# rneddojr/Adapting-Pretrained-Vision-Transformers-with-LoRA-against-Attack-Vectors

Hardware: AMD Instinct MI355X
Metric: adversarial images/sec (PGD-20, ViT-B/16+LoRA r=8, bs256) (higher is better)
Workload: dtype f16; 1 GPU; PGD-20 eps=8/255 alpha=2/255 random_start, ViT-B/16 (21 classes) + LoRA r=8 on q,k,v,attn-out,fc2 (fused), batch 256/GPU of synthetic 224x224x3 in HBM, seeded random-init weights; global_batch=256, per_gpu_batch=256, scaling=weak, pgd_steps=20, lora_rank=8, parallelism=dp1 (batch shards, no data-path collective), ranks_seen_by_collective=1

## Files before the change

adapting-pretrained-vision-transformers-with-lora-against-attack-vectors_amd/csrc/cls_path.hip:

```cpp
#include "kernels.h"
#include "prof.h"

namespace VLNS {

namespace {

constexpr int HD = 64;

__device__ __forceinline__ float row8_sum(float v) {
    v += __shfl_xor(v, 1, 64); v += __shfl_xor(v, 2, 64); return v + __shfl_xor(v, 4, 64);
}
__device__ __forceinline__ float slot8_sum(float v) {
    v += __shfl_xor(v, 8, 64); v += __shfl_xor(v, 16, 64); return v + __shfl_xor(v, 32, 64);
}
__device__ __forceinline__ float slot8_max(float v) {
    v = fmaxf(v, __shfl_xor(v, 8, 64)); v = fmaxf(v, __shfl_xor(v, 16, 64)); return fmaxf(v, __shfl_xor(v, 32, 64));
}
__device__ __forceinline__ void cvt8(const h16x8& t, float (&v)[8]) {
#pragma unroll
    for (int k = 0; k < 8; ++k) v[k] = h2f(t[k]);
}

__global__ __launch_bounds__(256) void attn_cls_fwd_kernel(const h16* __restrict__ qkv, h16* __restrict__ ctx_c,
                                                           float* __restrict__ lse_c, int B, int T, int H, int D,
// ... 120 lines not shown
    if (i >= (int64_t)B * n4) return;
    const int b = (int)(i / n4), c = (int)(i - (int64_t)b * n4);
    const h16x4 v = *(const h16x4*)(src + b * stride + 4 * c);
    *(f32x4*)(dst + (int64_t)b * D + 4 * c) = f32x4{h2f(v[0]), h2f(v[1]), h2f(v[2]), h2f(v[3])};
}
__global__ __launch_bounds__(256) void scatter_rows_kernel(const float* __restrict__ src, h16* __restrict__ dst, int B, int D,
                                                           int64_t stride) {
    const int n4 = D / 4;
    const int64_t i = blockIdx.x * (int64_t)blockDim.x + threadIdx.x;
    if (i >= (int64_t)B * n4) return;
    const int b = (int)(i / n4), c = (int)(i - (int64_t)b * n4);
    const f32x4 v = *(const f32x4*)(src + (int64_t)b * D + 4 * c);
    *(h16x4*)(dst + b * stride + 4 * c) = h16x4{f2h_sat(v[0]), f2h_sat(v[1]), f2h_sat(v[2]), f2h_sat(v[3])};
}

}

int k_attn_cls_fwd(const h16* qkv, h16* ctx_c, float* lse_c, int B, int T, int H, int D, hipStream_t s) {
    if (T > 256 || D != H * HD) return -1;
    ProfScope prof_("attn_cls_fwd_kernel", 4.0 * B * H * (double)T * HD, (double)B * T * D * 4.0, s);
    hipLaunchKernelGGL(attn_cls_fwd_kernel, dim3((B * H + 3) / 4), dim3(256), 0, s, qkv, ctx_c, lse_c, B, T, H, D,
                       0.125f * 1.4426950408889634f);
    return 0;
}
int k_attn_cls_bwd(const h16* qkv, const h16* ctx_c, const h16* dctx_c, const float* lse_c, h16* dqkv, int B, int T, int H, int D,
                   hipStream_t s) {
    if (T > 256 || D != H * HD) return -1;
    ProfScope prof_("attn_cls_bwd_kernel", 10.0 * B * H * (double)T * HD, (double)B * T * D * 10.0, s);
    hipLaunchKernelGGL(attn_cls_bwd_kernel, dim3((B * H + 3) / 4), dim3(256), 0, s, qkv, ctx_c, dctx_c, lse_c, dqkv, B, T, H, D,
                       0.125f, 0.125f * 1.4426950408889634f);
    return 0;
}
void k_gather_rows(const h16* src, float* dst, int B, int D, int64_t stride, hipStream_t s) {
    const int64_t n = (int64_t)B * (D / 4);
    hipLaunchKernelGGL(gather_rows_kernel, dim3((unsigned)((n + 255) / 256)), dim3(256), 0, s, src, dst, B, D, stride);
}
void k_scatter_rows(const float* src, h16* dst, int B, int D, int64_t stride, hipStream_t s) {
    const int64_t n = (int64_t)B * (D / 4);
    hipLaunchKernelGGL(scatter_rows_kernel, dim3((unsigned)((n + 255) / 256)), dim3(256), 0, s, src, dst, B, D, stride);
}

}
```

adapting-pretrained-vision-transformers-with-lora-against-attack-vectors_amd/csrc/kernels.h:

```cpp
#pragma once
#include "common.h"
#include "gemm.h"

namespace VLNS {

void k_patch_gather(const float* x, h16* out, int B, int S, int P, int normalise, const float* mean,
                    const float* std, hipStream_t s);
void k_cls_rows(float* x, const float* cls, const float* pos, int B, int T, int D, hipStream_t s);
void k_layernorm_fwd(const float* x, h16* h, float* mean, float* rstd, const float* g, const float* b, int M, int D,
                     float eps, const h16* delta, float* xout, const h16* P, int ng, h16* t, hipStream_t s,
                     int ldh = 0);
void k_layernorm_bwd(const h16* dh, const float* x, const float* mean, const float* rstd, const float* g,
                     const float* dres, float* dx, h16* dx_h, int M, int D, const h16* P, int ng, h16* u, hipStream_t s,
                     int* err = nullptr, int ldh = 0);
void k_head_fwd(const float* x, int B, int T, int D, int C, float eps, const float* g, const float* b, const float* Wc,
                const float* bc, float* xhat, float* xf, float* rstd, float* logits, hipStream_t s);
void k_cls_rows16(h16* x, const float* cls, const float* pos, int B, int T, int D, hipStream_t s);
void k_layernorm_fwd16(const h16* x, h16* h, float* mean, float* rstd, const float* g, const float* b, int M, int D,
                       float eps, const h16* delta, h16* xout, const h16* P, int ng, h16* t, hipStream_t s, int* err = nullptr);
void k_layernorm_bwd16(const h16* dh, const h16* x, const float* mean, const float* rstd, const float* g, h16* dres, int M, int D,
                       const h16* P, int ng, h16* u, hipStream_t s, int* err = nullptr);
void k_head_fwd16(const h16* x, int B, int T, int D, int C, float eps, const float* g, const float* b, const float* Wc,
                  const float* bc, float* xhat, float* xf, float* rstd, float* logits, hipStream_t s);
void k_ce_loss(const float* logits, const int64_t* labels, int B, int C, float* dlogits, float* loss_img, float* loss,
// ... 79 lines not shown

void attention32_set_ring(int on);
int attention32_init(int device);
int k_attention32_fwd(const h16* qkv, h16* ctx, float* lse2, int B, int T, int H, int D, hipStream_t s);
int k_attention32_bwd(const h16* qkv, const h16* ctx, const h16* dctx, const float* lse2, h16* dqkv, int B, int T,
                      int H, int D, hipStream_t s);

int k_attention_img_fwd(const h16* qkv, h16* ctx, float* lse2, int B, int T, int H, int D, const h16* Ad, h16* t, int r,
                        hipStream_t s);
int k_attention_img_bwd(const h16* qkv, const h16* ctx, const h16* dctx, const float* lse2, h16* dqkv, int B, int T, int H,
                        int D, const h16* Bd, h16* u, int r, unsigned mods, hipStream_t s, int force_ring = -1);

int k_attn_cls_fwd(const h16* qkv, h16* ctx_c, float* lse_c, int B, int T, int H, int D, hipStream_t s);
int k_attn_cls_bwd(const h16* qkv, const h16* ctx_c, const h16* dctx_c, const float* lse_c, h16* dqkv, int B, int T, int H, int D,
                   hipStream_t s);
void k_gather_rows(const h16* src, float* dst, int B, int D, int64_t stride, hipStream_t s);
void k_scatter_rows(const float* src, h16* dst, int B, int D, int64_t stride, hipStream_t s);

void k_patch_overlay(const float* img, const float* patch, const float* mats, const float* persp, float* out, int B, int S,
                     int ps, int circle, hipStream_t s);
void k_patch_overlay_bwd(const float* g, const float* mats, const float* persp, float* dpatch, int B, int S, int ps, int circle,
                         hipStream_t s);
void k_clamp(float* x, float lo, float hi, int64_t n, hipStream_t s);

int lora_wgrad_chunk(int M);
int lora_wgrad_chunks(int M);
void k_lora_wgrad(const h16* L, int ldl, int ncols_l, const h16* Rm, int ldr, int ncols_r, int M, float scale,
                  float* out, int ldo, int transpose_out, const float* inv_gscale, int64_t chunk_stride, hipStream_t s);
void k_reduce_chunks(const float* slab, float* out, int64_t n, int chunks, int64_t stride, hipStream_t s);

// ... 2 lines not shown
```

adapting-pretrained-vision-transformers-with-lora-against-attack-vectors_amd/csrc/model.h:

```cpp
#pragma once
#include <cstddef>
#include <string>
#include <vector>

#include "common.h"
#define vl_model VL_API(vl_model)
#include "../../include/vitlora.h"
#include "kernels.h"

enum { LQKV = 0, LO = 1, LFC1 = 2, LFC2 = 3 };
static const uint32_t kTargetBits[6] = {VL_T_Q, VL_T_K, VL_T_V, VL_T_O, VL_T_FC1, VL_T_FC2};

namespace VLNS {

struct Slot {
    int target_idx;
    int row_off;
    int out, in;
    int ext_off;
    int64_t a_off, b_off;
};

struct Linear {
    int out = 0, in = 0;
// ... 30 lines not shown
    std::vector<h16*> t[4];
    float *xhat, *xf, *rstd_f, *logits, *dlogits, *loss, *loss_img;
    float *gscale, *inv_gscale;
    float* dres[2];
    h16 *dres_h;
    h16 *dh, *dctx, *dqkv, *dz, *u;
    h16* xd;
    float* wg_slab;
    float* grad_img;
    struct Cls {
        int64_t Bc = 0;
        float *x0, *x1, *x2, *mean, *rstd, *lse;
        h16 *ctx, *delta, *h2, *a, *z, *t;
        float* dres[2];
        h16 *dres_h, *dh, *dctx, *dz, *u;
    } c;
    float *stage_x0, *stage_adv;
    int64_t* stage_labels;
    float* f_patches;
    std::vector<float*> f_h1, f_h2, f_a, f_qkv, f_ctx, f_z;
    std::vector<float*> f_t[4];
    float *f_dh, *f_dctx, *f_dqkv, *f_dz, *f_u, *f_xd, *f_tmp;
};

struct Pass {
    Workspace ws;
    int B = 0, rows = 0;
    int norm = 0, train = 0, cls_only = 0, have_loss = 0;
};

// ... 43 lines not shown
    hipStream_t cap_stream = nullptr;
    static constexpr int CHAIN_MAX_BATCH = 191;
    VLNS::Pass half[2];
    int chain_batch = 0;
    int pgd_chains = 0;
    hipStream_t side_stream = nullptr;
    hipEvent_t ev_fork = nullptr, ev_join = nullptr;
    int api_chains = 0;
    int fwd_chains = 0;
    int64_t n_captures = 0, n_commits = 0;
    int use_graph = 1;
    int resid_epi = 2;
    int plan_batch = 0, plan_train = 0;
    int attn_img_mode = -1;
    int num_cus = 256;
    int dead_rows = 1;
    int fuse_down_min_k = 2048;
    int small_m_rows = 16384;
    int fuse_pgd = 1;
    int square_bare = 0;
    int* err_flag = nullptr;
    float mean[3] = {0.485f, 0.456f, 0.406f};
    float stdv[3] = {0.229f, 0.224f, 0.225f};
};

static_assert(offsetof(vl_model, cfg) == 0, "api_dispatch.cpp reads the precision through the vl_config the handle starts with");

int vl_fail(int code, const char* fmt, ...);
#define HIPCHK(expr)                                                                            \
    do {                                                                                        \
// ... 40 lines not shown
```

adapting-pretrained-vision-transformers-with-lora-against-attack-vectors_amd/csrc/vitlora.hip:

```cpp
#include <algorithm>
#include <cstdarg>
#include <cstdio>
#include <cstdlib>
#include <cstring>
#include <string>
#include <vector>

#include "common.h"
#include "env.h"
#include "api_rename.h"
#include "model.h"
#include "prof.h"

extern std::vector<VlFlatRecord> g_vl_models;
extern long long g_poison_count;
#ifndef VL_BF16
Profiler* g_prof = nullptr;
int g_poison_lds = 0;
long long g_poison_count = 0;
namespace {
__global__ __launch_bounds__(256) void poison_lds_kernel(unsigned pattern, unsigned* sink) {
    extern __shared__ unsigned lds_all[];
    constexpr int N = 160 * 1024 / 4;
    for (int i = threadIdx.x; i < N; i += 256) lds_all[i] = pattern;
// ... 139 lines not shown
            launch_gemm(main, EPI_STORE_H16, 128, s);
            GemmArgs lo = gemm_args(u, ln.kext, ln.Au, ln.kext, ln.kext, Mpad, ln.in);
            lo.Mvalid = Mvalid; lo.k2_algo = 0;
            lo.C = g.C; lo.ldc = g.ldc; lo.R = p.ws.xd; lo.ldr = ln.in;
            if (epi == EPI_GELU_BWD) { lo.G = (const h16*)g.R; lo.ldg = g.ldr; }
            lo.drop_seed = m->drop_seed; lo.drop_stream = stream_id; lo.drop_p = m->cfg.lora_dropout;
            lo.drop_inv_keep = 1.f / (1.f - m->cfg.lora_dropout);
            launch_gemm(lo, EPI_DROP_ACC, 128, s);
            return;
        }
        g.k2_algo = m->r * (int)ln.slots.size();
        g.k2_used = ext_cols(m, ln);
        add_ext(g, u, ln.kext, ln.Au, ln.kext, ln.kext);
    }
    launch_gemm(g, epi, 128, s);
}

int parse_layer(const char* name, const char** rest) {
    const char* pfx = "vit.encoder.layer.";
    const size_t n = strlen(pfx);
    if (strncmp(name, pfx, n) != 0) return -1;
    char* end = nullptr;
    long i = strtol(name + n, &end, 10);
    if (end == name + n || *end != '.') return -1;
    *rest = end + 1;
    return (int)i;
}

bool capturing(hipStream_t s) {
    hipStreamCaptureStatus st = hipStreamCaptureStatusNone;
// ... 75 lines not shown
    if (int e = gemm_init(dev)) return fail(VL_ERR_HIP, "gemm_init: hipFuncSetAttribute failed (%d) on device %d", e, dev);
    if (int e = attention32_init(dev)) return fail(VL_ERR_HIP, "attention32_init: hipFuncSetAttribute failed (%d) on device %d", e, dev);
    if (int e = f32_init(dev)) return fail(VL_ERR_HIP, "f32_init: hipFuncSetAttribute failed (%d) on device %d", e, dev);
    vl_model* m = new vl_model();
    m->cfg = *cfg;
    m->device = dev;
    m->f32 = cfg->precision == VL_PREC_F32;
    m->D = cfg->hidden; m->L = cfg->layers; m->H = cfg->heads; m->MLP = cfg->mlp;
    m->S = cfg->image_size; m->P = cfg->patch_size; m->G = G; m->NP = G * G; m->T = G * G + 1;
    m->C = cfg->num_labels; m->PK = 3 * cfg->patch_size * cfg->patch_size;
    m->r = cfg->lora_targets ? cfg->lora_r : 0;
    m->scaling = m->r ? cfg->lora_alpha / (float)m->r : 0.f;
    m->use_graph = !env_flag("VITLORA_NO_GRAPH", false);
    m->resid_epi = env_resid();
    m->dead_rows = env_flag("VITLORA_DEAD_ROWS", true);
    m->fuse_pgd = env_flag("VITLORA_FUSE_PGD", true);
    m->pgd_chains = std::min(std::max(env_int("VITLORA_PGD_CHAINS", m->pgd_chains), 0), 2);
    m->fuse_down_min_k = env_int("VITLORA_FUSE_DOWN_MIN_K", m->fuse_down_min_k);
    m->small_m_rows = env_int("VITLORA_SMALL_M_ROWS", m->small_m_rows);
    m->attn_img_mode = env_attn_img();
    { hipDeviceProp_t prop; m->num_cus = hipGetDeviceProperties(&prop, dev) == hipSuccess ? prop.multiProcessorCount : 256; }
    const int D = m->D, MLP = m->MLP, r = m->r;
    int rc;
#define A_(p, n) if ((rc = dev_alloc(m, &(p), (size_t)(n))) != VL_OK) { vl_destroy(m); return rc; }
    const bool f32 = m->f32;
    if (f32) { A_(m->Wpe_f32, (size_t)D * m->PK); } else { A_(m->Wpe, (size_t)D * m->PK); A_(m->WpeT, (size_t)m->PK * D); }
    A_(m->bpe, D); A_(m->cls, D);
    A_(m->pos, (size_t)m->T * D); A_(m->lnf_g, D); A_(m->lnf_b, D);
    int64_t off = 0;
    m->layers.resize(m->L);
// ... 199 lines not shown
    m->dirty = 1;
    return VL_OK;
}

int vl_merge_weight(vl_model* m, int layer, uint32_t target, const float* W_in, float* W_out, void* stream) {
    if (!m || !W_in || !W_out) return fail(VL_ERR_ARG, "null argument");
    if (layer < 0 || layer >= m->L) return fail(VL_ERR_ARG, "layer out of range");
    for (int k = 0; k < 4; ++k)
        for (const Slot& sl : m->layers[layer].lin[k].slots)
            if (kTargetBits[sl.target_idx] == target) {
                k_merge_f32(W_in, m->flat + sl.a_off, m->flat + sl.b_off, sl.out, sl.in, m->r, m->scaling, W_out,
                            (hipStream_t)stream);
                return VL_OK;
            }
    return fail(VL_ERR_ARG, "target 0x%x has no adapter in layer %d", target, layer);
}

static size_t carve(const vl_model* m, Workspace& w, int B, int train, char* base) {
    const int D = m->D, L = m->L, MLP = m->MLP;
    const int64_t Mpad = pad_rows(m, B), Mppad = pad_patch_rows(m, B);
    Carver cv{base, 0};
    w.base = base; w.max_batch = base ? B : 0; w.train = train;
    w.Mpad = Mpad; w.Mppad = Mppad;
    w.xs.assign(2 * L + 1, nullptr); w.xs16.assign(2 * L + 1, nullptr);
    if (m->f32) for (auto& p : w.xs) p = cv.take<float>((size_t)Mpad * D * 4);
    else for (auto& p : w.xs16) p = cv.take<h16>((size_t)Mpad * D * 2);
    w.mean.resize(2 * L); w.rstd.resize(2 * L);
    for (int i = 0; i < 2 * L; ++i) { w.mean[i] = cv.take<float>(Mpad * 4); w.rstd[i] = cv.take<float>(Mpad * 4); }
    w.lse.resize(L);
    for (int l = 0; l < L; ++l) w.lse[l] = cv.take<float>((size_t)B * m->H * m->T * 4);
// ... 36 lines not shown
        c.lse = cv.take<float>((size_t)B * m->H * 4);
        c.ctx = cv.take<h16>((size_t)Bc * D * 2); c.delta = cv.take<h16>((size_t)Bc * D * 2); c.h2 = cv.take<h16>((size_t)Bc * D * 2);
        c.a = cv.take<h16>((size_t)Bc * MLP * 2); c.z = cv.take<h16>((size_t)Bc * MLP * 2);
        c.t = cv.take<h16>((size_t)Bc * kext_max * 2);
        c.dres[0] = cv.take<float>((size_t)Bc * D * 4); c.dres[1] = cv.take<float>((size_t)Bc * D * 4);
        c.dres_h = cv.take<h16>((size_t)Bc * D * 2); c.dh = cv.take<h16>((size_t)Bc * D * 2); c.dctx = cv.take<h16>((size_t)Bc * D * 2);
        c.dz = cv.take<h16>((size_t)Bc * MLP * 2); c.u = cv.take<h16>((size_t)Bc * kext_max * 2);
    }
    w.dres_h = cv.take<h16>((size_t)Mpad * D * 2);
    w.dh = cv.take<h16>((size_t)Mpad * D * 2);
    w.dctx = cv.take<h16>((size_t)Mpad * D * 2);
    w.dqkv = cv.take<h16>((size_t)Mpad * 3 * D * 2);
    w.dz = cv.take<h16>((size_t)Mpad * MLP * 2);
    w.u = cv.take<h16>((size_t)Mpad * kext_max * 2);
    w.xd = train ? cv.take<h16>((size_t)Mpad * MLP * 2) : nullptr;
    w.wg_slab = train && m->cls_w_off > 0 ? cv.take<float>((size_t)lora_wgrad_chunks((int)((int64_t)B * m->T)) * (size_t)m->cls_w_off * 4) : nullptr;
    return w.bytes = cv.off;
}
static size_t carve_bytes(const vl_model* m, int B, int train) {
    Workspace scratch;
    return carve(m, scratch, B, train, nullptr);
}

static int chain_images(const vl_model* m, int max_batch) {
    if (m->f32 || m->pgd_chains == 1 || max_batch < 2) return 0;
    const int top = max_batch < vl_model::CHAIN_MAX_BATCH ? max_batch : vl_model::CHAIN_MAX_BATCH;
    return (top + 1) / 2;
}

int vl_plan(vl_model* m, int max_batch, int train, size_t* bytes) {
// ... 49 lines not shown
        p.B = B; p.norm = normalise; p.have_loss = 0;
        return VL_OK;
    }
    k_patch_gather(x, w.patches, B, m->S, m->P, normalise, m->mean, m->stdv, s);
    {
        GemmArgs g = gemm_args(w.patches, m->PK, m->Wpe, m->PK, m->PK, Mppad, D);
        g.Mvalid = B * m->NP; g.bias = m->bpe; g.C = w.xs16[0]; g.ldc = D;
        g.pos = m->pos; g.tokens = T; g.patches = m->NP;
        launch_gemm(g, EPI_PATCH_FWD, 128, s);
    }
    k_cls_rows16(w.xs16[0], m->cls, m->pos, B, T, D, s);
    h16* delta = w.dres_h;
    int* const ef = m->err_flag;
    const bool re = m->resid_epi >= 1, re2 = m->resid_epi >= 2;
    const bool cls_only = m->dead_rows && !train;
    for (int l = 0; l < L; ++l) {
        Layer& ly = m->layers[l];
        GemmArgs g;
        const int n1 = fused_down_fwd(m, p, ly.lin[LQKV]);
        const h16* P1 = n1 ? ly.lin[LQKV].Ad : nullptr;
        if (l == 0 || re2) k_layernorm_fwd16(w.xs16[2 * l], w.h1[l], w.mean[2 * l], w.rstd[2 * l], ly.ln1_g, ly.ln1_b, M, D, m->cfg.ln_eps, nullptr, nullptr, P1, n1, w.t[LQKV][l], s, ef);
        else k_layernorm_fwd16(w.xs16[2 * l - 1], w.h1[l], w.mean[2 * l], w.rstd[2 * l], ly.ln1_g, ly.ln1_b, M, D, m->cfg.ln_eps, delta, w.xs16[2 * l], P1, n1, w.t[LQKV][l], s, ef);
        memset(&g, 0, sizeof g); g.C = w.qkv[l]; g.ldc = 3 * D;
        linear_fwd(m, p, ly.lin[LQKV], w.h1[l], w.t[LQKV][l], Mpad, M, g, EPI_STORE_H16, s, l * 4 + LQKV, n1 > 0);
        if (cls_only && l == L - 1) {
            Workspace::Cls& c = w.c;
            const int Bc = (int)c.Bc;
            if (k_attn_cls_fwd(w.qkv[l], c.ctx, c.lse, B, T, m->H, D, s)) return fail(VL_ERR_UNSUPPORTED, "attention: T > 256");
            memset(&g, 0, sizeof g); g.C = c.delta; g.ldc = D;
            linear_fwd(m, p, ly.lin[LO], c.ctx, c.t, Bc, B, g, EPI_STORE_H16, s, l * 4 + LO);
            k_gather_rows(w.xs16[2 * l], c.x0, B, D, (int64_t)T * D, s);
            const int n2c = fused_down_fwd(m, p, ly.lin[LFC1]);
            k_layernorm_fwd(c.x0, c.h2, c.mean, c.rstd, ly.ln2_g, ly.ln2_b, B, D, m->cfg.ln_eps, c.delta, c.x1,
                            n2c ? ly.lin[LFC1].Ad : nullptr, n2c, c.t, s);
            memset(&g, 0, sizeof g); g.C = c.a; g.ldc = m->MLP; g.C2 = c.z; g.ldc2 = m->MLP;
            linear_fwd(m, p, ly.lin[LFC1], c.h2, c.t, Bc, B, g, EPI_GELU, s, l * 4 + LFC1, n2c > 0);
            memset(&g, 0, sizeof g); g.C = c.delta; g.ldc = D;
            linear_fwd(m, p, ly.lin[LFC2], c.a, c.t, Bc, B, g, EPI_STORE_H16, s, l * 4 + LFC2);
            k_layernorm_fwd(c.x1, nullptr, nullptr, nullptr, nullptr, nullptr, B, D, m->cfg.ln_eps, c.delta, c.x2, nullptr, 0, nullptr, s);
            k_head_fwd(c.x2, B, 1, D, m->C, m->cfg.ln_eps, m->lnf_g, m->lnf_b, m->flat + m->cls_w_off,
                       m->flat + m->cls_b_off, w.xhat, w.xf, w.rstd_f, w.logits, s);
            p.B = B; p.norm = normalise; p.have_loss = 0; p.cls_only = 1;
            return VL_OK;
        }
        const bool img = attn_img(m, B);
        const bool t_o = img && down_fusable(m, ly.lin[LO]) && !vl_drop_on(m, p);
        if (img) {
            if (k_attention_img_fwd(w.qkv[l], w.ctx[l], w.lse[l], B, T, m->H, D, t_o ? ly.lin[LO].Ad : nullptr, w.t[LO][l], m->r, s))
                return fail(VL_ERR_UNSUPPORTED, "attention: T > 224");
        } else if (k_attention32_fwd(w.qkv[l], w.ctx[l], w.lse[l], B, T, m->H, D, s)) return fail(VL_ERR_UNSUPPORTED, "attention: T > 224");
        memset(&g, 0, sizeof g); g.C = delta; g.ldc = D;
        if (re) { g.C = w.xs16[2 * l + 1]; g.R = w.xs16[2 * l]; g.ldr = D; }
        linear_fwd(m, p, ly.lin[LO], w.ctx[l], w.t[LO][l], Mpad, M, g, re ? EPI_RESID_H16 : EPI_STORE_H16, s, l * 4 + LO, t_o);
        const int n2 = fused_down_fwd(m, p, ly.lin[LFC1]);
        const h16* P2 = n2 ? ly.lin[LFC1].Ad : nullptr;
        if (re) k_layernorm_fwd16(w.xs16[2 * l + 1], w.h2[l], w.mean[2 * l + 1], w.rstd[2 * l + 1], ly.ln2_g, ly.ln2_b, M, D, m->cfg.ln_eps, nullptr, nullptr, P2, n2, w.t[LFC1][l], s, ef);
        else k_layernorm_fwd16(w.xs16[2 * l], w.h2[l], w.mean[2 * l + 1], w.rstd[2 * l + 1], ly.ln2_g, ly.ln2_b, M, D, m->cfg.ln_eps, delta, w.xs16[2 * l + 1], P2, n2, w.t[LFC1][l], s, ef);
// ... 94 lines not shown
    for (int l = L - 1; l >= 0; --l) {
        Layer& ly = m->layers[l];
        GemmArgs g;
        if (cls_only && l == L - 1) {
            Workspace::Cls& c = w.c;
            const int Bc = (int)c.Bc;
            k_head_bwd(w.dlogits, w.gscale, m->flat + m->cls_w_off, m->lnf_g, w.xhat, w.rstd_f, B, 1, D, m->C, c.dres[0], c.dres_h, s);
            memset(&g, 0, sizeof g); g.C = c.dz; g.ldc = MLP; g.R = c.z; g.ldr = MLP;
            linear_dgrad(m, p, ly.lin[LFC2], c.dres_h, c.u, Bc, B, g, EPI_GELU_BWD, s, l * 4 + LFC2);
            memset(&g, 0, sizeof g); g.C = c.dh; g.ldc = D;
            linear_dgrad(m, p, ly.lin[LFC1], c.dz, c.u, Bc, B, g, EPI_STORE_H16, s, l * 4 + LFC1);
            const int foc = fused_down(m, ly.lin[LO]);
            k_layernorm_bwd(c.dh, c.x1, c.mean, c.rstd, ly.ln2_g, c.dres[0], c.dres[1], c.dres_h, B, D, ly.lin[LO].Bd, foc, c.u, s, m->err_flag);
            memset(&g, 0, sizeof g); g.C = c.dctx; g.ldc = D;
            linear_dgrad(m, p, ly.lin[LO], c.dres_h, c.u, Bc, B, g, EPI_STORE_H16, s, l * 4 + LO, foc > 0);
            if (k_attn_cls_bwd(w.qkv[l], c.ctx, c.dctx, c.lse, w.dqkv, B, T, m->H, D, s)) return fail(VL_ERR_UNSUPPORTED, "attention: T > 256");
            memset(&g, 0, sizeof g); g.C = w.dh; g.ldc = D;
            linear_dgrad(m, p, ly.lin[LQKV], w.dqkv, w.u, Mpad, M, g, EPI_STORE_H16, s, l * 4 + LQKV);
            k_zero(w.dres_h, (size_t)Mpad * D * sizeof(h16), s);
            k_scatter_rows(c.dres[1], w.dres_h, B, D, (int64_t)T * D, s);
            const int ffc = l > 0 ? fused_down(m, m->layers[l - 1].lin[LFC2]) : 0;
            k_layernorm_bwd16(w.dh, w.xs16[2 * l], w.mean[2 * l], w.rstd[2 * l], ly.ln1_g, w.dres_h,
                              M, D, ffc ? m->layers[l - 1].lin[LFC2].Bd : nullptr, ffc, w.u, s, m->err_flag);
            continue;
        }
        memset(&g, 0, sizeof g); g.C = w.dz; g.ldc = MLP; g.R = w.z[l]; g.ldr = MLP;
        linear_dgrad(m, p, ly.lin[LFC2], w.dres_h, w.u, Mpad, M, g, EPI_GELU_BWD, s, l * 4 + LFC2, l < L - 1 && fused_down(m, ly.lin[LFC2]) > 0);
        wgrad(ly.lin[LFC2], w.dres_h, w.a[l], w.t[LFC2][l], w.u, l * 4 + LFC2);
        memset(&g, 0, sizeof g); g.C = w.dh; g.ldc = D;
        linear_dgrad(m, p, ly.lin[LFC1], w.dz, w.u, Mpad, M, g, EPI_STORE_H16, s, l * 4 + LFC1);
        wgrad(ly.lin[LFC1], w.dz, w.h2[l], w.t[LFC1][l], w.u, l * 4 + LFC1);
        const int fo = fused_down(m, ly.lin[LO]);
        k_layernorm_bwd16(w.dh, w.xs16[2 * l + 1], w.mean[2 * l + 1], w.rstd[2 * l + 1], ly.ln2_g, w.dres_h, M, D, ly.lin[LO].Bd, fo, w.u, s,
// ... 472 lines not shown
    if (rc) return fail(VL_ERR_UNSUPPORTED, "attention kernel %d refused T %d", k, T);
    if (!capturing(s)) return check_launch("vl_debug_attention");
    return VL_OK;
}

int vl_debug_set_cus(vl_model* m, int cus) {
    if (cus <= 0) return fail(VL_ERR_ARG, "cus must be positive");
    gemm256_set_cus(cus); gemm_pp_set_cus(cus); gemm_stream_set_cus(cus);
    if (m) m->num_cus = cus;
    return VL_OK;
}

int vl_debug_set_option(vl_model* m, const char* name, int value) {
    if (!m || !name) return fail(VL_ERR_ARG, "null argument");
    if (!strcmp(name, "dead_rows")) m->dead_rows = value ? 1 : 0;
    else if (!strcmp(name, "fuse_pgd")) m->fuse_pgd = value ? 1 : 0;
    else if (!strcmp(name, "resid_epi")) m->resid_epi = value < 0 ? 0 : value > 2 ? 2 : value;
    else if (!strcmp(name, "attn_ring")) attention32_set_ring(value);
    else if (!strcmp(name, "poison_lds")) g_poison_lds = value ? 1 : 0;
    else if (!strcmp(name, "square_bare")) m->square_bare = value ? 1 : 0;
    else if (!strcmp(name, "pgd_chains")) m->pgd_chains = value < 0 ? 0 : value > 2 ? 2 : value;
    else if (!strcmp(name, "api_chains")) m->api_chains = value ? 1 : 0;
    else return fail(VL_ERR_ARG, "unknown option %s", name);
    drop_graphs(m);
    return VL_OK;
}

#ifndef VL_BF16
int vl_debug_set_gemm_pp(int mode) { const int old = gemm_pp_mode(); gemm_pp_set_mode(mode); return old; }
#endif
// ... 100 lines not shown
```

Baseline: 512.5 img/s.

## Skip last-layer K/V projection by folding CLS query into weights

In the last layer only the CLS row is needed. This path therefore no longer computes the full QKV projection over all tokens. It projects the CLS query and maps it back through Wk^T to get a per-head query in input space, then attends directly over the LN1 outputs. The value projection is applied afterwards to the B*H head-weighted sums, and the backward pass mirrors this with dedicated kernels. The goal is to remove a large M=B*T by 3D GEMM in the last layer, at the cost of extra small GEMMs, new custom kernels, and buffers carved out of the existing workspace.

```diff
diff --git a/adapting-pretrained-vision-transformers-with-lora-against-attack-vectors_amd/csrc/cls_path.hip b/adapting-pretrained-vision-transformers-with-lora-against-attack-vectors_amd/csrc/cls_path.hip
--- a/adapting-pretrained-vision-transformers-with-lora-against-attack-vectors_amd/csrc/cls_path.hip
+++ b/adapting-pretrained-vision-transformers-with-lora-against-attack-vectors_amd/csrc/cls_path.hip
@@ -158,6 +158,185 @@
     *(h16x4*)(dst + b * stride + 4 * c) = h16x4{f2h_sat(v[0]), f2h_sat(v[1]), f2h_sat(v[2]), f2h_sat(v[3])};
 }
 
+constexpr int KV_THREADS = 512;
+constexpr int KV_TMAX = 224;
+typedef float f32x2 __attribute__((ext_vector_type(2)));
+
+__device__ __forceinline__ float wave_sum(float v) {
+#pragma unroll
+    for (int o = 32; o > 0; o >>= 1) v += __shfl_xor(v, o, 64);
+    return v;
+}
+__device__ __forceinline__ float wave_max(float v) {
+#pragma unroll
+    for (int o = 32; o > 0; o >>= 1) v = fmaxf(v, __shfl_xor(v, o, 64));
+    return v;
+}
+
+__device__ __forceinline__ void kv_head_dots(const h16* __restrict__ h, const h16* __restrict__ rows, float (*S)[KV_TMAX], int T, int H,
+                                             int D) {
+    const int lane = threadIdx.x & 63, w = threadIdx.x >> 6;
+    const int fr = lane & 15, fg = lane >> 4;
+    const h16* rp = rows + (size_t)min(fr, H - 1) * D + fg * 8;
+    for (int tile = w; tile * 16 < T; tile += KV_THREADS / 64) {
+        const h16* hp = h + (size_t)min(tile * 16 + fr, T - 1) * D + fg * 8;
+        f32x4 acc = {0.f, 0.f, 0.f, 0.f};
+#pragma unroll 4
+        for (int k0 = 0; k0 < D; k0 += 32) acc = mfma16(*(const h16x8*)(rp + k0), *(const h16x8*)(hp + k0), acc);
+#pragma unroll
+        for (int i = 0; i < 4; ++i) S[fg * 4 + i][tile * 16 + fr] = acc[i];
+    }
+}
+
+template <int NH>
+__global__ __launch_bounds__(KV_THREADS) void cls_kv_fwd_kernel(const h16* __restrict__ h, const h16* __restrict__ qt,
+                                                                float* __restrict__ p, h16* __restrict__ hb, int T, int H, int D,
+                                                                float scale_log2e) {
+    __shared__ float S[16][KV_TMAX];
+    __shared__ __attribute__((aligned(16))) float P[KV_TMAX][NH];
+    const int b = blockIdx.x, tid = threadIdx.x, lane = tid & 63, w = tid >> 6;
+    h += (size_t)b * T * D; qt += (size_t)b * H * D; p += (size_t)b * H * T; hb += (size_t)b * H * D;
+    for (int i = tid; i < KV_TMAX * NH; i += KV_THREADS) (&P[0][0])[i] = 0.f;
+    kv_head_dots(h, qt, S, T, H, D);
+    __syncthreads();
+    for (int a = w; a < H; a += KV_THREADS / 64) {
+        float v[4], mx = -INFINITY, l = 0.f;
+#pragma unroll
+        for (int i = 0; i < 4; ++i) { const int j = lane + 64 * i; v[i] = j < T ? S[a][j] : -INFINITY; mx = fmaxf(mx, v[i]); }
+        mx = wave_max(mx);
+#pragma unroll
+        for (int i = 0; i < 4; ++i) { v[i] = lane + 64 * i < T ? __builtin_amdgcn_exp2f((v[i] - mx) * scale_log2e) : 0.f; l += v[i]; }
+        const float inv = 1.f / wave_sum(l);
+#pragma unroll
+        for (int i = 0; i < 4; ++i) {
+            const int j = lane + 64 * i;
+            if (j < T) { P[j][a] = v[i] * inv; p[(size_t)a * T + j] = v[i] * inv; }
+        }
+    }
+    __syncthreads();
+    if (2 * tid >= D) return;
+    f32x2 acc[NH];
+#pragma unroll
+    for (int a = 0; a < NH; ++a) acc[a] = f32x2{0.f, 0.f};
+    const h16* hp = h + 2 * tid;
+    for (int j = 0; j < T; ++j) {
+        const h16x2 hv = *(const h16x2*)(hp + (size_t)j * D);
+        const f32x2 hf = {h2f(hv[0]), h2f(hv[1])};
+#pragma unroll
+        for (int a4 = 0; a4 < NH; a4 += 4) {
+            const f32x4 pv = *(const f32x4*)&P[j][a4];
+#pragma unroll
+            for (int e = 0; e < 4; ++e) acc[a4 + e] += pv[e] * hf;
+        }
+    }
+#pragma unroll
+    for (int a = 0; a < NH; ++a)
+        if (a < H) *(h16x2*)(hb + (size_t)a * D + 2 * tid) = h16x2{f2h(acc[a][0]), f2h(acc[a][1])};
+}
+
+template <int NH>
+__global__ __launch_bounds__(KV_THREADS) void cls_kv_bwd_kernel(const h16* __restrict__ h, const float* __restrict__ p,
+                                                                const h16* __restrict__ qt, const h16* __restrict__ g,
+                                                                h16* __restrict__ dh, float* __restrict__ dh0, h16* __restrict__ dqt,
+                                                                int T, int H, int D, float scale) {
+    __shared__ float S[16][KV_TMAX];
+    __shared__ __attribute__((aligned(16))) float C[KV_TMAX][2 * NH];
+    const int b = blockIdx.x, tid = threadIdx.x, lane = tid & 63, w = tid >> 6;
+    h += (size_t)b * T * D; qt += (size_t)b * H * D; g += (size_t)b * H * D; p += (size_t)b * H * T;
+    dh += (size_t)b * T * D; dh0 += (size_t)b * D; dqt += (size_t)b * H * D;
+    for (int i = tid; i < KV_TMAX * 2 * NH; i += KV_THREADS) (&C[0][0])[i] = 0.f;
+    kv_head_dots(h, g, S, T, H, D);
+    __syncthreads();
+    for (int a = w; a < H; a += KV_THREADS / 64) {
+        float pv[4], dp[4], dl = 0.f;
+#pragma unroll
+        for (int i = 0; i < 4; ++i) {
+            const int j = lane + 64 * i;
+            pv[i] = j < T ? p[(size_t)a * T + j] : 0.f;
+            dp[i] = j < T ? S[a][j] : 0.f;
+            dl = fmaf(pv[i], dp[i], dl);
+        }
+        dl = wave_sum(dl);
+#pragma unroll
+        for (int i = 0; i < 4; ++i) {
+            const int j = lane + 64 * i;
+            if (j < T) { C[j][a] = pv[i]; C[j][NH + a] = pv[i] * (dp[i] - dl) * scale; }
+        }
+    }
+    __syncthreads();
+    if (2 * tid >= D) return;
+    f32x2 gv[NH], qv[NH], acc[NH];
+#pragma unroll
+    for (int a = 0; a < NH; ++a) {
+        acc[a] = gv[a] = qv[a] = f32x2{0.f, 0.f};
+        if (a < H) {
+            const h16x2 g2 = *(const h16x2*)(g + (size_t)a * D + 2 * tid), q2 = *(const h16x2*)(qt + (size_t)a * D + 2 * tid);
+            gv[a] = f32x2{h2f(g2[0]), h2f(g2[1])};
+            qv[a] = f32x2{h2f(q2[0]), h2f(q2[1])};
+        }
+    }
+    const h16* hp = h + 2 * tid;
+    for (int j = 0; j < T; ++j) {
+        const h16x2 hv = *(const h16x2*)(hp + (size_t)j * D);
+        const f32x2 hf = {h2f(hv[0]), h2f(hv[1])};
+        f32x2 o = {0.f, 0.f};
+#pragma unroll
+        for (int a4 = 0; a4 < NH; a4 += 4) {
+            const f32x4 pv = *(const f32x4*)&C[j][a4], dv = *(const f32x4*)&C[j][NH + a4];
+#pragma unroll
+            for (int e = 0; e < 4; ++e) {
+                o += pv[e] * gv[a4 + e];
+                o += dv[e] * qv[a4 + e];
+                acc[a4 + e] += dv[e] * hf;
+            }
+        }
+        if (j == 0) *(f32x2*)(dh0 + 2 * tid) = o;
+        else *(h16x2*)(dh + (size_t)j * D + 2 * tid) = h16x2{f2h(o[0]), f2h(o[1])};
+    }
+#pragma unroll
+    for (int a = 0; a < NH; ++a)
+        if (a < H) *(h16x2*)(dqt + (size_t)a * D + 2 * tid) = h16x2{f2h(acc[a][0]), f2h(acc[a][1])};
+}
+
+__global__ __launch_bounds__(256) void cls_gather16_kernel(const h16* __restrict__ src, h16* __restrict__ dst, int B, int D,
+                                                           int64_t stride) {
+    const int n8 = D / 8;
+    const int64_t i = blockIdx.x * (int64_t)blockDim.x + threadIdx.x;
+    if (i >= (int64_t)B * n8) return;
+    const int b = (int)(i / n8), c = (int)(i - (int64_t)b * n8);
+    *(h16x8*)(dst + (int64_t)b * D + 8 * c) = *(const h16x8*)(src + b * stride + 8 * c);
+}
+__global__ __launch_bounds__(256) void cls_expand_kernel(const h16* __restrict__ src, h16* __restrict__ dst, int B, int H, int D) {
+    const int n8 = D / 8;
+    const int64_t i = blockIdx.x * (int64_t)blockDim.x + threadIdx.x;
+    if (i >= (int64_t)B * H * n8) return;
+    const int row = (int)(i / n8), c = (int)(i - (int64_t)row * n8);
+    const int b = row / H, a = row - b * H;
+    h16x8 v;
+#pragma unroll
+    for (int e = 0; e < 8; ++e) v[e] = (h16)0.f;
+    if (c / (HD / 8) == a) v = *(const h16x8*)(src + (int64_t)b * D + 8 * c);
+    *(h16x8*)(dst + (int64_t)row * D + 8 * c) = v;
+}
+__global__ __launch_bounds__(256) void cls_pick_kernel(const h16* __restrict__ src, h16* __restrict__ dst, int B, int H, int D) {
+    const int n8 = D / 8;
+    const int64_t i = blockIdx.x * (int64_t)blockDim.x + threadIdx.x;
+    if (i >= (int64_t)B * n8) return;
+    const int b = (int)(i / n8), c = (int)(i - (int64_t)b * n8);
+    const int a = c / (HD / 8);
+    *(h16x8*)(dst + (int64_t)b * D + 8 * c) = *(const h16x8*)(src + ((int64_t)b * H + a) * D + 8 * c);
+}
+__global__ __launch_bounds__(256) void cls_add_row0_kernel(const float* __restrict__ x, const h16* __restrict__ y,
+                                                           h16* __restrict__ dh, int B, int D, int64_t stride) {
+    const int n4 = D / 4;
+    const int64_t i = blockIdx.x * (int64_t)blockDim.x + threadIdx.x;
+    if (i >= (int64_t)B * n4) return;
+    const int b = (int)(i / n4), c = (int)(i - (int64_t)b * n4);
+    const h16x4 q = *(const h16x4*)(y + (int64_t)b * D + 4 * c);
+    const f32x4 v = *(const f32x4*)(x + (int64_t)b * D + 4 * c) + f32x4{h2f(q[0]), h2f(q[1]), h2f(q[2]), h2f(q[3])};
+    *(h16x4*)(dh + b * stride + 4 * c) = h16x4{f2h(v[0]), f2h(v[1]), f2h(v[2]), f2h(v[3])};
+}
+
 }
 
 int k_attn_cls_fwd(const h16* qkv, h16* ctx_c, float* lse_c, int B, int T, int H, int D, hipStream_t s) {
@@ -175,6 +354,45 @@
                        0.125f, 0.125f * 1.4426950408889634f);
     return 0;
 }
+bool k_cls_kv_supported(int T, int H, int D) { return T >= 1 && T <= KV_TMAX && H >= 1 && H <= 16 && D == H * HD && D <= 2 * KV_THREADS; }
+int k_cls_kv_fwd(const h16* h, const h16* qt, float* p, h16* hb, int B, int T, int H, int D, hipStream_t s) {
+    if (!k_cls_kv_supported(T, H, D)) return -1;
+    ProfScope prof_("cls_kv_fwd_kernel", 4.0 * B * H * (double)T * D, (double)B * T * D * 2.0 + (double)B * H * (4.0 * D + 4.0 * T), s);
+    const float sl = 0.125f * 1.4426950408889634f;
+    if (H <= 4) hipLaunchKernelGGL(cls_kv_fwd_kernel<4>, dim3(B), dim3(KV_THREADS), 0, s, h, qt, p, hb, T, H, D, sl);
+    else if (H <= 12) hipLaunchKernelGGL(cls_kv_fwd_kernel<12>, dim3(B), dim3(KV_THREADS), 0, s, h, qt, p, hb, T, H, D, sl);
+    else hipLaunchKernelGGL(cls_kv_fwd_kernel<16>, dim3(B), dim3(KV_THREADS), 0, s, h, qt, p, hb, T, H, D, sl);
+    return 0;
+}
+int k_cls_kv_bwd(const h16* h, const float* p, const h16* qt, const h16* g, h16* dh, float* dh0, h16* dqt, int B, int T, int H, int D,
+                 hipStream_t s) {
+    if (!k_cls_kv_supported(T, H, D)) return -1;
+    ProfScope prof_("cls_kv_bwd_kernel", 8.0 * B * H * (double)T * D, (double)B * T * D * 4.0 + (double)B * H * (6.0 * D + 4.0 * T), s);
+    if (H <= 4) hipLaunchKernelGGL(cls_kv_bwd_kernel<4>, dim3(B), dim3(KV_THREADS), 0, s, h, p, qt, g, dh, dh0, dqt, T, H, D, 0.125f);
+    else if (H <= 12) hipLaunchKernelGGL(cls_kv_bwd_kernel<12>, dim3(B), dim3(KV_THREADS), 0, s, h, p, qt, g, dh, dh0, dqt, T, H, D, 0.125f);
+    else hipLaunchKernelGGL(cls_kv_bwd_kernel<16>, dim3(B), dim3(KV_THREADS), 0, s, h, p, qt, g, dh, dh0, dqt, T, H, D, 0.125f);
+    return 0;
+}
+void k_cls_gather16(const h16* src, h16* dst, int B, int D, int64_t stride, hipStream_t s) {
+    ProfScope prof_("cls_gather16_kernel", 0.0, (double)B * D * 4.0, s);
+    const int64_t n = (int64_t)B * (D / 8);
+    hipLaunchKernelGGL(cls_gather16_kernel, dim3((unsigned)((n + 255) / 256)), dim3(256), 0, s, src, dst, B, D, stride);
+}
+void k_cls_expand(const h16* src, h16* dst, int B, int H, int D, hipStream_t s) {
+    ProfScope prof_("cls_expand_kernel", 0.0, (double)B * D * 2.0 + (double)B * H * D * 2.0, s);
+    const int64_t n = (int64_t)B * H * (D / 8);
+    hipLaunchKernelGGL(cls_expand_kernel, dim3((unsigned)((n + 255) / 256)), dim3(256), 0, s, src, dst, B, H, D);
+}
+void k_cls_pick(const h16* src, h16* dst, int B, int H, int D, hipStream_t s) {
+    ProfScope prof_("cls_pick_kernel", 0.0, (double)B * D * 4.0, s);
+    const int64_t n = (int64_t)B * (D / 8);
+    hipLaunchKernelGGL(cls_pick_kernel, dim3((unsigned)((n + 255) / 256)), dim3(256), 0, s, src, dst, B, H, D);
+}
+void k_cls_add_row0(const float* x, const h16* y, h16* dh, int B, int D, int64_t stride, hipStream_t s) {
+    ProfScope prof_("cls_add_row0_kernel", (double)B * D, (double)B * D * 8.0, s);
+    const int64_t n = (int64_t)B * (D / 4);
+    hipLaunchKernelGGL(cls_add_row0_kernel, dim3((unsigned)((n + 255) / 256)), dim3(256), 0, s, x, y, dh, B, D, stride);
+}
 void k_gather_rows(const h16* src, float* dst, int B, int D, int64_t stride, hipStream_t s) {
     const int64_t n = (int64_t)B * (D / 4);
     hipLaunchKernelGGL(gather_rows_kernel, dim3((unsigned)((n + 255) / 256)), dim3(256), 0, s, src, dst, B, D, stride);
diff --git a/adapting-pretrained-vision-transformers-with-lora-against-attack-vectors_amd/csrc/kernels.h b/adapting-pretrained-vision-transformers-with-lora-against-attack-vectors_amd/csrc/kernels.h
--- a/adapting-pretrained-vision-transformers-with-lora-against-attack-vectors_amd/csrc/kernels.h
+++ b/adapting-pretrained-vision-transformers-with-lora-against-attack-vectors_amd/csrc/kernels.h
@@ -117,6 +117,14 @@
 int k_attn_cls_fwd(const h16* qkv, h16* ctx_c, float* lse_c, int B, int T, int H, int D, hipStream_t s);
 int k_attn_cls_bwd(const h16* qkv, const h16* ctx_c, const h16* dctx_c, const float* lse_c, h16* dqkv, int B, int T, int H, int D,
                    hipStream_t s);
+bool k_cls_kv_supported(int T, int H, int D);
+int k_cls_kv_fwd(const h16* h, const h16* qt, float* p, h16* hb, int B, int T, int H, int D, hipStream_t s);
+int k_cls_kv_bwd(const h16* h, const float* p, const h16* qt, const h16* g, h16* dh, float* dh0, h16* dqt, int B, int T, int H, int D,
+                 hipStream_t s);
+void k_cls_gather16(const h16* src, h16* dst, int B, int D, int64_t stride, hipStream_t s);
+void k_cls_expand(const h16* src, h16* dst, int B, int H, int D, hipStream_t s);
+void k_cls_pick(const h16* src, h16* dst, int B, int H, int D, hipStream_t s);
+void k_cls_add_row0(const float* x, const h16* y, h16* dh, int B, int D, int64_t stride, hipStream_t s);
 void k_gather_rows(const h16* src, float* dst, int B, int D, int64_t stride, hipStream_t s);
 void k_scatter_rows(const float* src, h16* dst, int B, int D, int64_t stride, hipStream_t s);
 
diff --git a/adapting-pretrained-vision-transformers-with-lora-against-attack-vectors_amd/csrc/model.h b/adapting-pretrained-vision-transformers-with-lora-against-attack-vectors_amd/csrc/model.h
--- a/adapting-pretrained-vision-transformers-with-lora-against-attack-vectors_amd/csrc/model.h
+++ b/adapting-pretrained-vision-transformers-with-lora-against-attack-vectors_amd/csrc/model.h
@@ -68,6 +68,15 @@
         h16 *ctx, *delta, *h2, *a, *z, *t;
         float* dres[2];
         h16 *dres_h, *dh, *dctx, *dz, *u;
+        int64_t BHp = 0;
+        int kv_fits = 0;
+        h16 *h0, *q, *dq;
+        h16 *ex;
+        h16 *qt, *hb, *g, *dqt;
+        h16 *t2;
+        float *p;
+        float *dh0a;
+        h16 *dh0q;
     } c;
     float *stage_x0, *stage_adv;
     int64_t* stage_labels;
@@ -141,6 +150,8 @@
     int plan_batch = 0, plan_train = 0;
     int attn_img_mode = -1;
     int num_cus = 256;
+    int cls_kv = 1;
+    int cls_kv_min_rows = 16384;
     int dead_rows = 1;
     int fuse_down_min_k = 2048;
     int small_m_rows = 16384;
diff --git a/adapting-pretrained-vision-transformers-with-lora-against-attack-vectors_amd/csrc/vitlora.hip b/adapting-pretrained-vision-transformers-with-lora-against-attack-vectors_amd/csrc/vitlora.hip
--- a/adapting-pretrained-vision-transformers-with-lora-against-attack-vectors_amd/csrc/vitlora.hip
+++ b/adapting-pretrained-vision-transformers-with-lora-against-attack-vectors_amd/csrc/vitlora.hip
@@ -177,6 +177,45 @@
         add_ext(g, u, ln.kext, ln.Au, ln.kext, ln.kext);
     }
     launch_gemm(g, epi, 128, s);
+}
+
+bool module_down_inside(const vl_model* m, const Linear& ln, GemmArgs& g, const h16* down_W, int down_ldw, h16* down_out, int epi) {
+    if (ln.kext != 64) return false;
+    GemmArgs f = g;
+    f.down_W = down_W; f.down_ldw = down_ldw; f.down_out = down_out; f.down_ld = ln.kext;
+    f.down_groups = ext_cols(m, ln) <= 16 ? 1 : ext_cols(m, ln) <= 32 ? 2 : 0;
+    if (!f.down_groups || !gemm_pp_fuses_down(f, epi)) return false;
+    g = f; g.A2 = nullptr;
+    return true;
+}
+void module_fwd(const vl_model* m, const Linear& ln, int row0, const h16* x, h16* t, int Mpad, int Mvalid, h16* y, bool bias,
+                hipStream_t s) {
+    GemmArgs g = gemm_args(x, ln.in, ln.W + (size_t)row0 * ln.in, ln.in, ln.in, Mpad, m->D);
+    g.Mvalid = Mvalid; g.C = y; g.ldc = m->D; g.bias = bias ? ln.bias + row0 : nullptr;
+    if (ln.kext && !m->cfg.lora_merged) {
+        g.k2_algo = m->r; g.k2_used = ext_cols(m, ln);
+        add_ext(g, t, ln.kext, ln.Bu + (size_t)row0 * ln.kext, ln.kext, ln.kext);
+        if (!module_down_inside(m, ln, g, ln.Ad, ln.in, t, EPI_STORE_H16)) {
+            GemmArgs d = gemm_args(x, ln.in, ln.Ad, ln.in, ln.in, Mpad, ln.kext);
+            d.Mvalid = Mvalid; d.n_algo = m->r; d.C = t; d.ldc = ln.kext;
+            launch_gemm(d, EPI_STORE_H16, 64, s);
+        }
+    }
+    launch_gemm(g, EPI_STORE_H16, 128, s);
+}
+void module_dgrad(const vl_model* m, const Linear& ln, int row0, const h16* dy, h16* u, int Mpad, int Mvalid, h16* dx, hipStream_t s) {
+    GemmArgs g = gemm_args(dy, m->D, ln.WT + row0, ln.out, m->D, Mpad, ln.in);
+    g.Mvalid = Mvalid; g.C = dx; g.ldc = ln.in;
+    if (ln.kext && !m->cfg.lora_merged) {
+        g.k2_algo = m->r; g.k2_used = ext_cols(m, ln);
+        add_ext(g, u, ln.kext, ln.Au, ln.kext, ln.kext);
+        if (!module_down_inside(m, ln, g, ln.Bd + row0, ln.out, u, EPI_STORE_H16)) {
+            GemmArgs d = gemm_args(dy, m->D, ln.Bd + row0, ln.out, m->D, Mpad, ln.kext);
+            d.Mvalid = Mvalid; d.n_algo = m->r; d.C = u; d.ldc = ln.kext;
+            launch_gemm(d, EPI_STORE_H16, 64, s);
+        }
+    }
+    launch_gemm(g, EPI_STORE_H16, 128, s);
 }
 
 int parse_layer(const char* name, const char** rest) {
@@ -282,6 +321,7 @@
     m->use_graph = !env_flag("VITLORA_NO_GRAPH", false);
     m->resid_epi = env_resid();
     m->dead_rows = env_flag("VITLORA_DEAD_ROWS", true);
+    m->cls_kv = std::min(std::max(env_int("VITLORA_CLS_KV", m->cls_kv), 0), 2);
     m->fuse_pgd = env_flag("VITLORA_FUSE_PGD", true);
     m->pgd_chains = std::min(std::max(env_int("VITLORA_PGD_CHAINS", m->pgd_chains), 0), 2);
     m->fuse_down_min_k = env_int("VITLORA_FUSE_DOWN_MIN_K", m->fuse_down_min_k);
@@ -511,6 +551,31 @@
                 return VL_OK;
             }
     return fail(VL_ERR_ARG, "target 0x%x has no adapter in layer %d", target, layer);
+}
+
+static void place_cls_kv(const vl_model* m, Workspace& w, int B, int kext_max) {
+    Workspace::Cls& c = w.c;
+    const int D = m->D, L = m->L;
+    const size_t Bc = (size_t)c.Bc, BHp = (size_t)round_up((int64_t)B * m->H, 256), rows = (size_t)w.Mpad;
+    c.BHp = (int64_t)BHp; c.kv_fits = 0;
+    if (!w.base) return;
+    struct Region { char* p; size_t n; };
+    bool ok = true;
+    auto take = [&ok](Region* r, size_t bytes) -> char* {
+        bytes = (size_t)round_up((int64_t)bytes, 256);
+        for (int i = 0; i < 3; ++i)
+            if (r[i].n >= bytes) { char* p = r[i].p; r[i].p += bytes; r[i].n -= bytes; return p; }
+        ok = false;
+        return nullptr;
+    };
+    Region f[3] = {{(char*)w.qkv[L - 1], rows * 3 * D * 2}, {(char*)w.ctx[L - 1], rows * D * 2}, {(char*)w.z[L - 1], rows * m->MLP * 2}};
+    c.qt = (h16*)take(f, BHp * D * 2); c.ex = (h16*)take(f, BHp * D * 2); c.hb = (h16*)take(f, BHp * D * 2);
+    c.t2 = (h16*)take(f, BHp * kext_max * 2); c.h0 = (h16*)take(f, Bc * D * 2); c.q = (h16*)take(f, Bc * D * 2);
+    c.p = (float*)take(f, (size_t)B * m->H * m->T * 4);
+    c.dqt = c.hb; c.dq = c.q; c.dh0q = c.h0;
+    Region b[3] = {{(char*)w.dqkv, rows * 3 * D * 2}, {(char*)w.dctx, rows * D * 2}, {(char*)w.dz, rows * m->MLP * 2}};
+    c.g = (h16*)take(b, BHp * D * 2); c.dh0a = (float*)take(b, Bc * D * 4);
+    c.kv_fits = ok ? 1 : 0;
 }
 
 static size_t carve(const vl_model* m, Workspace& w, int B, int train, char* base) {
@@ -577,6 +642,7 @@
     w.dz = cv.take<h16>((size_t)Mpad * MLP * 2);
     w.u = cv.take<h16>((size_t)Mpad * kext_max * 2);
     w.xd = train ? cv.take<h16>((size_t)Mpad * MLP * 2) : nullptr;
+    place_cls_kv(m, w, B, kext_max);
     w.wg_slab = train && m->cls_w_off > 0 ? cv.take<float>((size_t)lora_wgrad_chunks((int)((int64_t)B * m->T)) * (size_t)m->cls_w_off * 4) : nullptr;
     return w.bytes = cv.off;
 }
@@ -656,19 +722,34 @@
     int* const ef = m->err_flag;
     const bool re = m->resid_epi >= 1, re2 = m->resid_epi >= 2;
     const bool cls_only = m->dead_rows && !train;
+    const bool cls_kv = cls_only && w.c.kv_fits && k_cls_kv_supported(T, m->H, D) &&
+                        (m->cls_kv == 2 || (m->cls_kv == 1 && (int64_t)m->plan_batch * T > m->cls_kv_min_rows));
     for (int l = 0; l < L; ++l) {
         Layer& ly = m->layers[l];
         GemmArgs g;
-        const int n1 = fused_down_fwd(m, p, ly.lin[LQKV]);
+        const bool kv = cls_kv && l == L - 1;
+        const int n1 = kv ? 0 : fused_down_fwd(m, p, ly.lin[LQKV]);
         const h16* P1 = n1 ? ly.lin[LQKV].Ad : nullptr;
         if (l == 0 || re2) k_layernorm_fwd16(w.xs16[2 * l], w.h1[l], w.mean[2 * l], w.rstd[2 * l], ly.ln1_g, ly.ln1_b, M, D, m->cfg.ln_eps, nullptr, nullptr, P1, n1, w.t[LQKV][l], s, ef);
         else k_layernorm_fwd16(w.xs16[2 * l - 1], w.h1[l], w.mean[2 * l], w.rstd[2 * l], ly.ln1_g, ly.ln1_b, M, D, m->cfg.ln_eps, delta, w.xs16[2 * l], P1, n1, w.t[LQKV][l], s, ef);
-        memset(&g, 0, sizeof g); g.C = w.qkv[l]; g.ldc = 3 * D;
-        linear_fwd(m, p, ly.lin[LQKV], w.h1[l], w.t[LQKV][l], Mpad, M, g, EPI_STORE_H16, s, l * 4 + LQKV, n1 > 0);
+        if (!kv) {
+            memset(&g, 0, sizeof g); g.C = w.qkv[l]; g.ldc = 3 * D;
+            linear_fwd(m, p, ly.lin[LQKV], w.h1[l], w.t[LQKV][l], Mpad, M, g, EPI_STORE_H16, s, l * 4 + LQKV, n1 > 0);
+        }
         if (cls_only && l == L - 1) {
             Workspace::Cls& c = w.c;
             const int Bc = (int)c.Bc;
-            if (k_attn_cls_fwd(w.qkv[l], c.ctx, c.lse, B, T, m->H, D, s)) return fail(VL_ERR_UNSUPPORTED, "attention: T > 256");
+            if (kv) {
+                const Linear& lq = ly.lin[LQKV];
+                const int BH = B * m->H, BHp = (int)c.BHp;
+                k_cls_gather16(w.h1[l], c.h0, B, D, (int64_t)T * D, s);
+                module_fwd(m, lq, 0, c.h0, c.t, Bc, B, c.q, true, s);
+                k_cls_expand(c.q, c.ex, B, m->H, D, s);
+                module_dgrad(m, lq, D, c.ex, c.t2, BHp, BH, c.qt, s);
+                if (k_cls_kv_fwd(w.h1[l], c.qt, c.p, c.hb, B, T, m->H, D, s)) return fail(VL_ERR_UNSUPPORTED, "attention: T > 224");
+                module_fwd(m, lq, 2 * D, c.hb, c.t2, BHp, BH, c.ex, true, s);
+                k_cls_pick(c.ex, c.ctx, B, m->H, D, s);
+            } else if (k_attn_cls_fwd(w.qkv[l], c.ctx, c.lse, B, T, m->H, D, s)) return fail(VL_ERR_UNSUPPORTED, "attention: T > 256");
             memset(&g, 0, sizeof g); g.C = c.delta; g.ldc = D;
             linear_fwd(m, p, ly.lin[LO], c.ctx, c.t, Bc, B, g, EPI_STORE_H16, s, l * 4 + LO);
             k_gather_rows(w.xs16[2 * l], c.x0, B, D, (int64_t)T * D, s);
@@ -682,7 +763,7 @@
             k_layernorm_fwd(c.x1, nullptr, nullptr, nullptr, nullptr, nullptr, B, D, m->cfg.ln_eps, c.delta, c.x2, nullptr, 0, nullptr, s);
             k_head_fwd(c.x2, B, 1, D, m->C, m->cfg.ln_eps, m->lnf_g, m->lnf_b, m->flat + m->cls_w_off,
                        m->flat + m->cls_b_off, w.xhat, w.xf, w.rstd_f, w.logits, s);
-            p.B = B; p.norm = normalise; p.have_loss = 0; p.cls_only = 1;
+            p.B = B; p.norm = normalise; p.have_loss = 0; p.cls_only = kv ? 2 : 1;
             return VL_OK;
         }
         const bool img = attn_img(m, B);
@@ -807,9 +888,21 @@
             k_layernorm_bwd(c.dh, c.x1, c.mean, c.rstd, ly.ln2_g, c.dres[0], c.dres[1], c.dres_h, B, D, ly.lin[LO].Bd, foc, c.u, s, m->err_flag);
             memset(&g, 0, sizeof g); g.C = c.dctx; g.ldc = D;
             linear_dgrad(m, p, ly.lin[LO], c.dres_h, c.u, Bc, B, g, EPI_STORE_H16, s, l * 4 + LO, foc > 0);
-            if (k_attn_cls_bwd(w.qkv[l], c.ctx, c.dctx, c.lse, w.dqkv, B, T, m->H, D, s)) return fail(VL_ERR_UNSUPPORTED, "attention: T > 256");
-            memset(&g, 0, sizeof g); g.C = w.dh; g.ldc = D;
-            linear_dgrad(m, p, ly.lin[LQKV], w.dqkv, w.u, Mpad, M, g, EPI_STORE_H16, s, l * 4 + LQKV);
+            if (p.cls_only == 2) {
+                const Linear& lq = ly.lin[LQKV];
+                const int BH = B * m->H, BHp = (int)c.BHp;
+                k_cls_expand(c.dctx, c.ex, B, m->H, D, s);
+                module_dgrad(m, lq, 2 * D, c.ex, c.t2, BHp, BH, c.g, s);
+                if (k_cls_kv_bwd(w.h1[l], c.p, c.qt, c.g, w.dh, c.dh0a, c.dqt, B, T, m->H, D, s)) return fail(VL_ERR_UNSUPPORTED, "attention: T > 224");
+                module_fwd(m, lq, D, c.dqt, c.t2, BHp, BH, c.ex, false, s);
+                k_cls_pick(c.ex, c.dq, B, m->H, D, s);
+                module_dgrad(m, lq, 0, c.dq, c.u, Bc, B, c.dh0q, s);
+                k_cls_add_row0(c.dh0a, c.dh0q, w.dh, B, D, (int64_t)T * D, s);
+            } else {
+                if (k_attn_cls_bwd(w.qkv[l], c.ctx, c.dctx, c.lse, w.dqkv, B, T, m->H, D, s)) return fail(VL_ERR_UNSUPPORTED, "attention: T > 256");
+                memset(&g, 0, sizeof g); g.C = w.dh; g.ldc = D;
+                linear_dgrad(m, p, ly.lin[LQKV], w.dqkv, w.u, Mpad, M, g, EPI_STORE_H16, s, l * 4 + LQKV);
+            }
             k_zero(w.dres_h, (size_t)Mpad * D * sizeof(h16), s);
             k_scatter_rows(c.dres[1], w.dres_h, B, D, (int64_t)T * D, s);
             const int ffc = l > 0 ? fused_down(m, m->layers[l - 1].lin[LFC2]) : 0;
@@ -1312,6 +1405,7 @@
 int vl_debug_set_option(vl_model* m, const char* name, int value) {
     if (!m || !name) return fail(VL_ERR_ARG, "null argument");
     if (!strcmp(name, "dead_rows")) m->dead_rows = value ? 1 : 0;
+    else if (!strcmp(name, "cls_kv")) m->cls_kv = value < 0 ? 0 : value > 2 ? 2 : value;
     else if (!strcmp(name, "fuse_pgd")) m->fuse_pgd = value ? 1 : 0;
     else if (!strcmp(name, "resid_epi")) m->resid_epi = value < 0 ? 0 : value > 2 ? 2 : value;
     else if (!strcmp(name, "attn_ring")) attention32_set_ring(value);
```

Result: no change. 517.4 img/s, median of 6 (+1.0%).
